# ehsankharazmi/hp-VPINNs

Hardware: AMD Instinct MI355X
Metric: variational-loss iterations/sec (higher is better)
Workload: dtype f64; 1 GPU; Poisson-2D hp-VPINN, 16x16 elements, 20x20 GLL quad/elem, 10x10 test fcns/elem, MLP [2,20,20,20,1] tanh, var_form 1, 320 boundary pts, TF1 Adam (BASELINE config 4); points=102400, residuals=25600, params=921, backend=mfma, parallelism=element-sharded dp1, exchange=none, pass_structure=whole-iteration, kernel_variant=k_iter_fused<L=3,SPLIT=false,QT=true>

## Files before the change

### hp_vpinns_amd/csrc/kernels_fused.hip

```cpp
#include <cstdio>
#include <cstdlib>
#include <cstring>
#include <type_traits>

#include "hpv_mfma_dev.h"
#include "hpv_fused_dev.h"

#define FZ_WAVES 4
#define FZ_BLOCK (FZ_WAVES * 64)
#define FZ_PRE_PER_THREAD 4
#define FZ_C 3
#define FZ_SHAPE_CONSTS                                                                                              \
    static constexpr int FZ_QX = QX_, FZ_QY = QY_, FZ_NTX = NTX_, FZ_NTY = NTY_, FZ_NQ = QX_ * QY_, FZ_NR = NTX_ * NTY_; \
    static constexpr int FZ_TPE = FZ_NQ / 16;                                                                        \
    static constexpr int FZ_MAXT = FZ_TPE / 4 + 1;       \
    static_assert(FZ_NQ % 16 == 0 && FZ_TPE % 4 <= 1, "element shape not covered by the whole-iteration kernel");
#define FZ_SHAPES(X) X(20, 20, 10, 10) X(16, 16, 8, 8) X(12, 12, 6, 6)

#ifdef HPV_FZ_TIMING
#define FZ_STAMP(I) fz_t[I] = clock64()
#define FZ_SEG(I) do { const long long t_ = clock64(); fz_seg[I] += t_ - fz_last; fz_last = t_; } while (0)
#else
#define FZ_STAMP(I)
#define FZ_SEG(I)
// ... 517 lines not shown
        fwd_trip(k0, std::integral_constant<int, 2>{}, std::true_type{});
    } else {
#pragma unroll 1
        for (; k0 + 1 < n_own; k0 += 2) fwd_trip(k0, std::integral_constant<int, 2>{}, std::false_type{});
        if (k0 < n_own) fwd_trip(k0, std::integral_constant<int, 1>{}, std::false_type{});
    }
    FZ_STAMP(2);
    if constexpr (SPLIT) {
        constexpr int NITG = (2 * FZ_NQ * 2 + FZ_BLOCK - 1) / FZ_BLOCK;
        bool ok = true;
        if (!xstay) ok = xg_gather<NITG, FZ_BLOCK>(g.xg + el * (2 * FZ_NQ) * 2, 2 * FZ_NQ * 2, xtag, (unsigned*)(lds + M::CH), tid);
        const int timed_out = __syncthreads_or(ok ? 0 : 1);
        if (timed_out || xstay) {
            if (timed_out && tid == 0) __hip_atomic_store(g.xerr, 1, __ATOMIC_RELAXED, __HIP_MEMORY_SCOPE_AGENT);
            return;
        }
    }
    __syncthreads();
    FZ_STAMP(3);
    if constexpr (QT) {
        if (tid == 0 && dtile < g.ntiles)
            g.data_part[dtile - g.data_off / 16] = (lds[M::RED + 8] + lds[M::RED + 9]) + (lds[M::RED + 10] + lds[M::RED + 11]);
    }

    {
        int nax_e = FZ_NTX, nay_e = FZ_NTY;
        double nr_e = (double)rnr;
        if (pa.pd.nact) {
            nax_e = __builtin_amdgcn_readfirstlane(pa.pd.nact[e]);
            nay_e = __builtin_amdgcn_readfirstlane(pa.pd.nacty[e]);
            nr_e = (double)(nax_e * nay_e);
        }
        constexpr bool PJ_SCALAR = NT2 > 0 && FZ_NQ == 256;
        if constexpr (PJ_SCALAR) {
            static_assert(!GEN || (M::AX == M::TR && 4 <= M::TR_WAVE), "the d-epsilon partials live in wave 0's part of the transpose region (it reads them back itself)");
            for (int o = tid; o < 2 * FZ_QY * FZ_NTX; o += FZ_BLOCK) {
                const int t = o / (FZ_QY * FZ_NTX), j = (o / FZ_NTX) % FZ_QY, r = o % FZ_NTX;
                const double* ax = lds + M::AX + (t * FZ_NTX + r) * FZ_QX;
                const double* gr = lds + M::CH + t * FZ_NQ + j * FZ_QX;
                double acc = 0.0;
#pragma unroll
                for (int i = 0; i < FZ_QX; ++i) acc = fma(ax[i], gr[i], acc);
                lds[M::T + o] = acc;
            }
            __syncthreads();
            if (tid < 2 * FZ_NR) {
                const int t = tid / FZ_NR, o = tid % FZ_NR, kk = o / FZ_NTX, r = o % FZ_NTX;
                const double* by = lds + M::BY + (t * FZ_NTY + kk) * FZ_QY;
                const double* tt = lds + M::T + t * FZ_QY * FZ_NTX + r;
                double acc = 0.0;
#pragma unroll
                for (int j = 0; j < FZ_QY; ++j) acc = fma(by[j], tt[j * FZ_NTX], acc);
                lds[M::UP + tid] = (t == 0 ? pc0 : pc1) * acc;
            }
            __syncthreads();
            double sq = 0.0;
            const double sc = 2.0 / nr_e;
            [[maybe_unused]] double deps = 0.0;
            if (tid < FZ_NR) {
                const bool act = ro_r < nax_e && ro_k < nay_e;
                double u;
                if constexpr (GEN) {
                    const double u0 = lds[M::UP + tid], u1 = lds[M::UP + FZ_NR + tid];
                    u = fma(gm0, u0, gm1 * u1) - pF;
                    if (!act) u = 0.0;
                    deps = sc * u * fma(ge0, u0, ge1 * u1);
                } else {
                    u = (lds[M::UP + tid] + lds[M::UP + FZ_NR + tid]) - pF;
                    if (!act) u = 0.0;
                }
                lds[M::U + tid] = u;
                if (ro_on) pa.R[ro_idx] = u;
                sq = u * u;
            }
            if (wv < 2) {
                sq = group_sum<64>(sq);
                if (lane == 0) lds[M::RED + wv] = sq;
            }
            __syncthreads();
            if (tid == 0) pa.loss_e[e] = (lds[M::RED] + lds[M::RED + 1]) / nr_e;
            for (int o = tid; o < 2 * FZ_NTY * FZ_QX; o += FZ_BLOCK) {
                const int t = o / (FZ_NTY * FZ_QX), kk = (o / FZ_QX) % FZ_NTY, i = o % FZ_QX;
                const double* ax = lds + M::AX + t * FZ_NTX * FZ_QX + i;
                const double* ur = lds + M::U + kk * FZ_NTX;
                double acc = 0.0;
#pragma unroll
                for (int r = 0; r < FZ_NTX; ++r) acc = fma(ax[r * FZ_QX], ur[r], acc);
                if constexpr (GEN) lds[M::S + o] = acc * sc * (t == 0 ? pc0 * gm0 : pc1 * gm1);
                else lds[M::S + o] = acc * sc * (t == 0 ? pc0 : pc1);
            }
            __syncthreads();
            const int n_adj = (GEN && !gtwo) ? FZ_NQ : 2 * FZ_NQ;
            for (int o = tid; o < n_adj; o += FZ_BLOCK) {
                const int t = o / FZ_NQ, j = (o / FZ_QX) % FZ_QY, i = o % FZ_QX;
                const double* by = lds + M::BY + t * FZ_NTY * FZ_QY + j;
                const double* sr = lds + M::S + t * FZ_NTY * FZ_QX + i;
                double acc = 0.0;
#pragma unroll
                for (int kk = 0; kk < FZ_NTY; ++kk) acc = fma(by[kk * FZ_QY], sr[kk * FZ_QX], acc);
                if constexpr (GEN) { if (!gtwo) deps = fma(acc, lds[M::CH + FZ_NQ + o], deps); }
                lds[M::CH + o] = acc;
            }
            if constexpr (GEN) {
                if (pa.pd.has_eps) {
                    deps = group_sum<64>(deps);
                    if (lane == 0) lds[M::AX + wv] = deps;
                }
            }
            __syncthreads();
            if constexpr (GEN) {
                if (pa.pd.has_eps && tid == 0) pa.deps_e[e] = (lds[M::AX] + lds[M::AX + 1]) + (lds[M::AX + 2] + lds[M::AX + 3]);
            }
        } else {
            constexpr int PJ_NJT = (FZ_QY + 15) / 16, PJ_NIT = (FZ_QX + 15) / 16;
            constexpr int PJ_KX = FZ_QX / 4, PJ_KR = (FZ_NTX + 3) / 4, PJ_KK = (FZ_NTY + 3) / 4;
            static_assert(FZ_QX % 4 == 0 && FZ_QY % 4 == 0 && FZ_NTX <= 16 && FZ_NTY <= 16, "projection tiles: whole k-steps over the points, one tile of test functions");
            static_assert(2 * PJ_NJT * FZ_NR <= 2 * FZ_QY * FZ_NTX, "the partial sums of U fit the T array (T itself stays in registers)");
            for (int u = wv; u < 2 * PJ_NJT; u += FZ_WAVES) {
                const int t = u / PJ_NJT, jt = u % PJ_NJT;
                const bool jon = jt * 16 + pt < FZ_QY, ron = pt < FZ_NTX, kon = pt < FZ_NTY;
                const double* gr = lds + M::CH + t * FZ_NQ + (jon ? jt * 16 + pt : 0) * FZ_QX + q;
                const double* ax = lds + M::AX + (t * FZ_NTX + (ron ? pt : 0)) * FZ_QX + q;
                const double* by = lds + M::BY + (t * FZ_NTY + (kon ? pt : 0)) * FZ_QY + jt * 16 + q;
                double ga[PJ_KX], xa[PJ_KX], ya[4];
#pragma unroll
                for (int s = 0; s < PJ_KX; ++s) { ga[s] = gr[4 * s]; xa[s] = ax[4 * s]; }
#pragma unroll
                for (int v = 0; v < 4; ++v) ya[v] = by[jt * 16 + 4 * v < FZ_QY ? 4 * v : 0];
                v4d tt = v4d{0.0, 0.0, 0.0, 0.0};
#pragma unroll
                for (int s = 0; s < PJ_KX; ++s)
                    tt = __builtin_amdgcn_mfma_f64_16x16x4f64(jon ? ga[s] : 0.0, ron ? xa[s] : 0.0, tt, 0, 0, 0);
                v4d up = v4d{0.0, 0.0, 0.0, 0.0};
#pragma unroll
                for (int v = 0; v < 4; ++v)
                    if (jt * 16 + 4 * v < FZ_QY)
                        up = __builtin_amdgcn_mfma_f64_16x16x4f64(kon ? ya[v] : 0.0, tt[v], up, 0, 0, 0);
#pragma unroll
                for (int v = 0; v < 4; ++v)
                    if (q + 4 * v < FZ_NTY && ron) lds[M::T + u * FZ_NR + (q + 4 * v) * FZ_NTX + pt] = up[v];
            }
            pj_lds_barrier();
            double sq = 0.0;
            const double sc = 2.0 / nr_e;
            [[maybe_unused]] double deps = 0.0;
            auto up_t = [&](int t) -> double {
                double a = lds[M::T + t * PJ_NJT * FZ_NR + tid];
#pragma unroll
                for (int jt = 1; jt < PJ_NJT; ++jt) a += lds[M::T + (t * PJ_NJT + jt) * FZ_NR + tid];
                return a;
            };
            if (tid < FZ_NR) {
                const bool act = ro_r < nax_e && ro_k < nay_e;
                double u;
                if constexpr (GEN) {
                    const double u0 = pc0 * up_t(0), u1 = pc1 * up_t(1);
                    u = fma(gm0, u0, gm1 * u1) - pF;
                    if (!act) u = 0.0;
                    deps = sc * u * fma(ge0, u0, ge1 * u1);
                } else {
                    u = (pc0 * up_t(0) + pc1 * up_t(1)) - pF;
                    if (!act) u = 0.0;
                }
                lds[M::U + tid] = u;
                if (ro_on) pa.R[ro_idx] = u;
                sq = u * u;
            }
            if (wv < 2) {
                sq = group_sum<64>(sq);
                if (lane == 0) lds[M::RED + wv] = sq;
            }
            pj_lds_barrier();
            if (tid == 0) pa.loss_e[e] = (lds[M::RED] + lds[M::RED + 1]) / nr_e;
            const int n_adj = (GEN && !gtwo) ? PJ_NIT : 2 * PJ_NIT;
            for (int u = wv; u < n_adj; u += FZ_WAVES) {
                const int t = u / PJ_NIT, it = u % PJ_NIT;
                const int i = it * 16 + pt;
                const bool ion = i < FZ_QX, kon = pt < FZ_NTY;
                const double* ur = lds + M::U + (kon ? pt : 0) * FZ_NTX;
                const double* ax = lds + M::AX + t * FZ_NTX * FZ_QX + (ion ? i : 0);
                double ua[PJ_KR], xa[PJ_KR];
#pragma unroll
                for (int s = 0; s < PJ_KR; ++s) {
                    const int rc = 4 * s + q < FZ_NTX ? 4 * s + q : 0;
                    ua[s] = ur[rc]; xa[s] = ax[rc * FZ_QX];
                }
                v4d ss = v4d{0.0, 0.0, 0.0, 0.0};
#pragma unroll
                for (int s = 0; s < PJ_KR; ++s) {
                    const bool ron = 4 * s + q < FZ_NTX;
                    ss = __builtin_amdgcn_mfma_f64_16x16x4f64((kon && ron) ? ua[s] : 0.0, (ron && ion) ? xa[s] : 0.0, ss, 0, 0, 0);
                }
#pragma unroll
                for (int v = 0; v < 4; ++v) {
                    if constexpr (GEN) ss[v] = ss[v] * sc * (t == 0 ? pc0 * gm0 : pc1 * gm1);
                    else ss[v] = ss[v] * sc * (t == 0 ? pc0 : pc1);
                }
#pragma unroll
                for (int jt = 0; jt < PJ_NJT; ++jt) {
                    const int j = jt * 16 + pt;
                    const bool jon = j < FZ_QY;
                    const double* by = lds + M::BY + t * FZ_NTY * FZ_QY + (jon ? j : 0);
                    v4d gg = v4d{0.0, 0.0, 0.0, 0.0};
#pragma unroll
                    for (int v = 0; v < PJ_KK; ++v) {
                        const bool k4 = 4 * v + q < FZ_NTY;
                        const double b = by[(k4 ? 4 * v + q : 0) * FZ_QY];
                        gg = __builtin_amdgcn_mfma_f64_16x16x4f64((k4 && jon) ? b : 0.0, ss[v], gg, 0, 0, 0);
                    }
#pragma unroll
                    for (int v = 0; v < 4; ++v) {
                        const int jo = jt * 16 + q + 4 * v;
                        if (jo < FZ_QY && ion) {
                            const int o = jo * FZ_QX + i;
                            if constexpr (GEN) { if (!gtwo) deps = fma(gg[v], lds[M::CH + FZ_NQ + o], deps); }
                            lds[M::CH + t * FZ_NQ + o] = gg[v];
                        }
                    }
                }
            }
            if constexpr (GEN) {
                if (pa.pd.has_eps) {
                    deps = group_sum<64>(deps);
                    if (lane == 0) lds[M::UP + wv] = deps;
                }
            }
            __syncthreads();
            if constexpr (GEN) {
                constexpr int PJ_DW = (M::UP - M::TR) / M::TR_WAVE;
                static_assert(PJ_DW < FZ_WAVES && M::UP + FZ_WAVES - M::TR <= (PJ_DW + 1) * M::TR_WAVE, "the d-epsilon partials live in one wave's part of the transpose region");
                if (pa.pd.has_eps && tid == PJ_DW * 64) pa.deps_e[e] = (lds[M::UP] + lds[M::UP + 1]) + (lds[M::UP + 2] + lds[M::UP + 3]);
            }
        }
    }

    FZ_STAMP(4);
    double* TAB = lds + M::TR + wv * M::TR_WAVE;
#pragma unroll
    for (int i = 0; i < LH; ++i) { dWacc[i] = v4d{0.0, 0.0, 0.0, 0.0}; dS10[i] = 0.0; dS01[i] = 0.0; accC[i] = 0.0; }
    dbo = 0.0;
#pragma unroll
    for (int s = 0; s < MF_KS; ++s) {
        dWo[s] = 0.0; dW1[0][s] = 0.0; dW1[1][s] = 0.0;
#pragma unroll
        for (int i = 0; i < L; ++i) db[i][s] = 0.0;
    }

#ifdef HPV_FZ_TIMING
    fz_last = clock64();
    fz_n_own = n_own;
    for (int i = 0; i < 2 + 2 * L; ++i) fz_seg[i] = 0;
#endif
    auto rev_tile = [&](int k) {
#ifdef HPV_FZ_TIMING
        fz_last = clock64();
#endif
        const long tile = tile_of(k);
        const long p = tile * 16 + pt;
        const bool valid = p < g.N;
        const double x0 = valid ? g.X[p] : 0.0, x1 = valid ? g.X[g.N + p] : 0.0;
        int lofs = lane;
        asm volatile("" : "+v"(lofs));
        double sv[NSV];
        if (k < n_lds) {
            const double* pk = k == 0 ? PKw : PKw2;
            if constexpr (NT2 > 0) pk = lds + M::PK + (k == 0 ? wv : (k == 1 ? 4 + wv : 8 + (wv & 1))) * (NSV * 64) + lane;
#pragma unroll
            for (int j = 0; j < NSV; ++j) sv[j] = pk[j * 64];
        } else {
            switch (k - n_lds) {
#define FZ_FETCH(K) case K: if constexpr (K < NREG) acc_get_all<AFULL + K * 2 * NSV, NSV>(sv); break;
                case 0:
                    if constexpr (NREG < 1) {
                    } else if constexpr (NPART > 0) {
                        const double* pp = lds + M::PP + wv * (NPART * 64) + lane;
#pragma unroll
                        for (int j = 0; j < NPART; ++j) sv[j] = pp[j * 64];
                        acc_get_from<ABASE, NSV, NPART>(sv);
                    } else {
                        acc_get_all<ABASE, NSV>(sv);
                    }
                    break;
                FZ_FETCH(1) FZ_FETCH(2) FZ_FETCH(3) FZ_FETCH(4)
#undef FZ_FETCH
                default:
#pragma unroll
                    for (int j = 0; j < NSV; ++j) sv[j] = 0.0;
            }
        }
        double gb[C];
        if (k < n_el) {
            const int lp = (tbase + wv + k * FZ_WAVES) * 16 + pt;
            gb[0] = 0.0; gb[1] = lds[M::CH + lp]; gb[2] = lds[M::CH + FZ_NQ + lp];
            if constexpr (GEN) {
                const double g0 = gb[1], g1 = gb[2];
#pragma unroll
                for (int c = 1; c < C; ++c) gb[c] = fma(wa0(c), g0, wb1(c) * g1);
            }
        } else {
            gb[0] = gdat; gb[1] = 0.0; gb[2] = 0.0;
            if constexpr (NT2 > 0) gb[3] = 0.0;
        }
        if constexpr (NT2 == 0) {
        double zd[L][MF_KS];
#pragma unroll
        for (int s = 0; s < MF_KS; ++s)
            zd[0][s] = fma(gb[1], lds[M::W1O + (0 * MF_KS + s) * 64 + lofs], gb[2] * lds[M::W1O + (1 * MF_KS + s) * 64 + lofs]);
#pragma unroll
        for (int i = 1; i < L; ++i) {
            double hd[MF_KS];
#pragma unroll
            for (int s = 0; s < MF_KS; ++s) {
                const double a = sv[(i - 1) * MF_KS + s];
                hd[s] = (1.0 - a * a) * zd[i - 1][s];
            }
            fz_layer<false>(lds + M::WT + (i - 1) * MF_KS * 64, lds + M::WR + (i - 1) * MF_KS * 16, nullptr, lofs, hd, zd[i]);
        }

        FZ_SEG(0);
        double hbar[2][MF_KS], zbar[2][MF_KS];
#pragma unroll
        for (int s = 0; s < MF_KS; ++s) {
            const double a = sv[(L - 1) * MF_KS + s], a1 = 1.0 - a * a;
            const double wo = lds[M::W1O + (2 * MF_KS + s) * 64 + lofs];
            if (k >= n_el) dWo[s] = fma(a, gb[0], dWo[s]);
            dWo[s] = fma(a1, zd[L - 1][s], dWo[s]);
            hbar[0][s] = gb[0] * wo; hbar[1][s] = wo;
        }
        if (q == 0) dbo += gb[0];
        FZ_SEG(1);

#pragma unroll
        for (int i = L - 1; i >= 0; --i) {
#pragma unroll
            for (int s = 0; s < MF_KS; ++s) {
                const double a = sv[i * MF_KS + s];
                const double a1 = 1.0 - a * a, a2 = -2.0 * a * a1;
                zbar[1][s] = hbar[1][s] * a1;
                const double zb = hbar[0][s] * a1 + a2 * (hbar[1][s] * zd[i][s]);
                zbar[0][s] = zb;
                db[i][s] += zb;
            }
            if (i == 0) {
#pragma unroll
                for (int s = 0; s < MF_KS; ++s) {
                    dW1[0][s] += x0 * zbar[0][s] + gb[1] * zbar[1][s];
                    dW1[1][s] += x1 * zbar[0][s] + gb[2] * zbar[1][s];
                }
            } else {
                pj_wave_sync();
#pragma unroll
                for (int ch = 0; ch < 2; ++ch) {
                    double* TA = TAB + (2 * ch) * (MF_TRB * MF_LD);
                    double* TB = TA + MF_TRB * MF_LD;
#pragma unroll
                    for (int s = 0; s < MF_KS; ++s) {
                        const double a = sv[(i - 1) * MF_KS + s], a1 = 1.0 - a * a;
                        const double hv = ch == 0 ? a : a1 * zd[i - 1][s];
                        TA[(4 * s + q) * MF_LD + pt] = hv;
                        TB[(4 * s + q) * MF_LD + pt] = zbar[ch][s];
                    }
                }
#pragma unroll
                for (int ch = 0; ch < 2; ++ch) {
                    v4d acc = v4d{0.0, 0.0, 0.0, 0.0};
                    double h4 = 0.0;
                    const double* wrl = lds + M::WRB + (i - 1) * MF_KS * 16 + q * 4 + (lane & 3);
#pragma unroll
                    for (int s = 0; s < MF_KS; ++s) {
                        acc = __builtin_amdgcn_mfma_f64_16x16x4f64(lds[M::WN + ((i - 1) * MF_KS + s) * 64 + lofs], zbar[ch][s], acc, 0, 0, 0);
                        h4 = __builtin_amdgcn_mfma_f64_4x4x4f64(wrl[s * 16], zbar[ch][s], h4, 0, 0, 0);
                    }
#pragma unroll
                    for (int s = 0; s < 4; ++s) hbar[ch][s] = acc[s];
                    hbar[ch][4] = h4;
                }
                FZ_SEG(2 + 2 * (L - 1 - i));
                pj_wave_sync();
#pragma unroll
                for (int ch = 0; ch < 2; ++ch) {
                    const double* TA = TAB + (2 * ch) * (MF_TRB * MF_LD);
                    const double* TB = TA + MF_TRB * MF_LD;
                    double aF[4], bF[4], aS[4], bS[4];
#pragma unroll
                    for (int kk = 0; kk < 4; ++kk) {
                        aF[kk] = TA[pt * MF_LD + 4 * kk + q];
                        bF[kk] = TB[pt * MF_LD + 4 * kk + q];
                        aS[kk] = TA[(16 + (lane & 3)) * MF_LD + 4 * kk + q];
                        bS[kk] = TB[(16 + (lane & 3)) * MF_LD + 4 * kk + q];
                    }
#pragma unroll
                    for (int kk = 0; kk < 4; ++kk) {
                        dWacc[i - 1] = __builtin_amdgcn_mfma_f64_16x16x4f64(aF[kk], bF[kk], dWacc[i - 1], 0, 0, 0);
                        dS10[i - 1] = __builtin_amdgcn_mfma_f64_4x4x4f64(aS[kk], bF[kk], dS10[i - 1], 0, 0, 0);
                        dS01[i - 1] = __builtin_amdgcn_mfma_f64_4x4x4f64(bS[kk], aF[kk], dS01[i - 1], 0, 0, 0);
                    }
                    accC[i - 1] = __builtin_amdgcn_mfma_f64_4x4x4f64(TA[(16 + (lane & 3)) * MF_LD + (pt & 12) + q],
                                                                   TB[(16 + (lane & 3)) * MF_LD + (pt & 12) + q], accC[i - 1], 0, 0, 0);
                }
                FZ_SEG(3 + 2 * (L - 1 - i));
            }
        }
        } else {
        double zc[L][2][MF_KS];
        [[maybe_unused]] double zq[L][MF_KS];
        [[maybe_unused]] auto sq2 = [&](int i, int s) -> double { return fma(g.t2w[0], zc[i][0][s] * zc[i][0][s], g.t2w[1] * (zc[i][1][s] * zc[i][1][s])); };
#define ZC(I, CC, SS) zc[(I)][(CC)][(SS)]
#pragma unroll
        for (int s = 0; s < MF_KS; ++s) {
            zc[0][0][s] = lds[M::W1O + (0 * MF_KS + s) * 64 + lofs];
            zc[0][1][s] = lds[M::W1O + (1 * MF_KS + s) * 64 + lofs];
        }
#pragma unroll
        for (int i = 1; i < L; ++i) {
            double hx[MF_KS], hy[MF_KS];
            [[maybe_unused]] double hq[MF_KS];
#pragma unroll
            for (int s = 0; s < MF_KS; ++s) {
                const double a = sv[(i - 1) * MF_KS + s], a1 = 1.0 - a * a;
                hx[s] = a1 * ZC(i - 1, 0, s); hy[s] = a1 * ZC(i - 1, 1, s);
                if constexpr (NT2 > 0) hq[s] = (-2.0 * a * a1) * sq2(i - 1, s) + (i > 1 ? a1 * zq[i > 1 ? i - 1 : 0][s] : 0.0);
            }
            fz_layer<false>(lds + M::WT + (i - 1) * MF_KS * 64, lds + M::WR + (i - 1) * MF_KS * 16, nullptr, lofs, hx, zc[i][0]);
            fz_layer<false>(lds + M::WT + (i - 1) * MF_KS * 64, lds + M::WR + (i - 1) * MF_KS * 16, nullptr, lofs, hy, zc[i][1]);
            if constexpr (NT2 > 0) fz_layer<false>(lds + M::WT + (i - 1) * MF_KS * 64, lds + M::WR + (i - 1) * MF_KS * 16, nullptr, lofs, hq, zq[i]);
        }

        FZ_SEG(0);
        double hbar[C][MF_KS], zbar[C][MF_KS];
        [[maybe_unused]] auto hv3 = [&](int i, int s) -> double {
            const double a = sv[i * MF_KS + s], a1 = 1.0 - a * a;
            return (-2.0 * a * a1) * sq2(i, s) + (i > 0 ? a1 * zq[i][s] : 0.0);
        };
#pragma unroll
        for (int s = 0; s < MF_KS; ++s) {
            const double a = sv[(L - 1) * MF_KS + s], a1 = 1.0 - a * a;
            const double wo = lds[M::W1O + (2 * MF_KS + s) * 64 + lofs];
            if (k >= n_el) dWo[s] = fma(a, gb[0], dWo[s]);
            dWo[s] = fma(a1 * zc[L - 1][0][s], gb[1], dWo[s]);
            dWo[s] = fma(a1 * zc[L - 1][1][s], gb[2], dWo[s]);
            hbar[0][s] = gb[0] * wo; hbar[1][s] = gb[1] * wo; hbar[2][s] = gb[2] * wo;
            if constexpr (NT2 > 0) { dWo[s] = fma(hv3(L - 1, s), gb[3], dWo[s]); hbar[3][s] = gb[3] * wo; }
        }
        if (q == 0) dbo += gb[0];
        FZ_SEG(1);

#pragma unroll
        for (int i = L - 1; i >= 0; --i) {
#pragma unroll
            for (int s = 0; s < MF_KS; ++s) {
                const double a = sv[i * MF_KS + s];
                const double a1 = 1.0 - a * a, a2 = -2.0 * a * a1;
                zbar[1][s] = hbar[1][s] * a1;
                zbar[2][s] = hbar[2][s] * a1;
                double zb = hbar[0][s] * a1 + a2 * (hbar[1][s] * ZC(i, 0, s) + hbar[2][s] * ZC(i, 1, s));
                if constexpr (NT2 > 0) {
                    const double hb = hbar[3][s], a3 = -2.0 * a1 * (1.0 - 3.0 * a * a);
                    zbar[3][s] = hb * a1;
                    zbar[1][s] = fma(2.0 * hb * a2 * g.t2w[0], ZC(i, 0, s), zbar[1][s]);
                    zbar[2][s] = fma(2.0 * hb * a2 * g.t2w[1], ZC(i, 1, s), zbar[2][s]);
                    zb = fma(hb, a3 * sq2(i, s) + (i > 0 ? a2 * zq[i][s] : 0.0), zb);
                }
                zbar[0][s] = zb;
                db[i][s] += zb;
            }
            if (i == 0) {
#pragma unroll
                for (int s = 0; s < MF_KS; ++s) {
                    dW1[0][s] += x0 * zbar[0][s] + zbar[1][s];
                    dW1[1][s] += x1 * zbar[0][s] + zbar[2][s];
                }
            } else {
                pj_wave_sync();
                auto tr_put = [&](int c0) {
#pragma unroll
                    for (int cc = 0; cc < TRG; ++cc) {
                        const int ch = c0 + cc;
                        double* TA = TAB + (2 * cc) * (MF_TRB * MF_LD);
                        double* TB = TA + MF_TRB * MF_LD;
#pragma unroll
                        for (int s = 0; s < MF_KS; ++s) {
                            const double a = sv[(i - 1) * MF_KS + s], a1 = 1.0 - a * a;
                            double hv;
                            if constexpr (NT2 > 0) hv = ch == 0 ? a : (ch == 3 ? hv3(i - 1, s) : a1 * ZC(i - 1, ch == 3 ? 0 : ch - 1, s));
                            else hv = ch == 0 ? a : a1 * ZC(i - 1, ch - 1, s);
                            TA[(4 * s + q) * MF_LD + pt] = hv;
                            TB[(4 * s + q) * MF_LD + pt] = zbar[ch][s];
                        }
                    }
                };
                tr_put(0);
#pragma unroll
                for (int ch = 0; ch < C; ++ch) {
                    v4d acc = v4d{0.0, 0.0, 0.0, 0.0};
                    double h4 = 0.0;
                    const double* wrl = lds + M::WRB + (i - 1) * MF_KS * 16 + q * 4 + (lane & 3);
#pragma unroll
                    for (int s = 0; s < MF_KS; ++s) {
                        acc = __builtin_amdgcn_mfma_f64_16x16x4f64(lds[M::WN + ((i - 1) * MF_KS + s) * 64 + lofs], zbar[ch][s], acc, 0, 0, 0);
                        h4 = __builtin_amdgcn_mfma_f64_4x4x4f64(wrl[s * 16], zbar[ch][s], h4, 0, 0, 0);
                    }
#pragma unroll
                    for (int s = 0; s < 4; ++s) hbar[ch][s] = acc[s];
                    hbar[ch][4] = h4;
                }
                FZ_SEG(2 + 2 * (L - 1 - i));
                pj_wave_sync();
                auto tr_mul = [&]() {
#pragma unroll
                    for (int ch = 0; ch < TRG; ++ch) {
                        const double* TA = TAB + (2 * ch) * (MF_TRB * MF_LD);
                        const double* TB = TA + MF_TRB * MF_LD;
                        double aF[4], bF[4], aS[4], bS[4];
#pragma unroll
                        for (int kk = 0; kk < 4; ++kk) {
                            aF[kk] = TA[pt * MF_LD + 4 * kk + q];
                            bF[kk] = TB[pt * MF_LD + 4 * kk + q];
                            aS[kk] = TA[(16 + (lane & 3)) * MF_LD + 4 * kk + q];
                            bS[kk] = TB[(16 + (lane & 3)) * MF_LD + 4 * kk + q];
                        }
#pragma unroll
                        for (int kk = 0; kk < 4; ++kk) {
                            dWacc[i - 1] = __builtin_amdgcn_mfma_f64_16x16x4f64(aF[kk], bF[kk], dWacc[i - 1], 0, 0, 0);
                            dS10[i - 1] = __builtin_amdgcn_mfma_f64_4x4x4f64(aS[kk], bF[kk], dS10[i - 1], 0, 0, 0);
                            dS01[i - 1] = __builtin_amdgcn_mfma_f64_4x4x4f64(bS[kk], aF[kk], dS01[i - 1], 0, 0, 0);
                        }
                        accC[i - 1] = __builtin_amdgcn_mfma_f64_4x4x4f64(TA[(16 + (lane & 3)) * MF_LD + (pt & 12) + q],
                                                                       TB[(16 + (lane & 3)) * MF_LD + (pt & 12) + q], accC[i - 1], 0, 0, 0);
                    }
                };
                tr_mul();
#pragma unroll
                for (int c0 = TRG; c0 < C; c0 += TRG) {
                    pj_wave_sync();
                    tr_put(c0);
                    pj_wave_sync();
                    tr_mul();
                }
                FZ_SEG(3 + 2 * (L - 1 - i));
            }
        }
        }
        FZ_SEG(1 + 2 * L);
    };
#undef ZC
#pragma unroll 1
    for (int k = 0; k < n_own; ++k) rev_tile(k);

    if constexpr (QT) {
        int lofs = lane;
        asm volatile("" : "+v"(lofs));
        const double X0 = g.X[q_p], X1 = g.X[g.N + q_p];
        double AAq[NSV];
#pragma unroll
        for (int j = 0; j < NSV; ++j) AAq[j] = PKQ[j * 32 + q_ci];
        const double mval = q_tan ? 0.0 : 1.0;
        double gch = lds[M::CH + (q_tan ? (qcs - 1) * FZ_NQ : 0) + q_lp];
        if constexpr (GEN && !DQ) {
            const double g0 = lds[M::CH + q_lp], g1 = lds[M::CH + FZ_NQ + q_lp];
            gch = qcs == 1 ? fma(wa0(1), g0, wb1(1) * g1) : fma(wa0(2), g0, wb1(2) * g1);
        }
        const double GB = q_tan ? (DQ ? 0.0 : gch) : (qcs == 3 ? gdat_q : 0.0);
        double Hq[L][MF_KS], ZCq[L][MF_KS];
#pragma unroll
        for (int s = 0; s < MF_KS; ++s) {
            const double w0 = lds[M::W1O + (0 * MF_KS + s) * 64 + lofs], w1 = lds[M::W1O + (1 * MF_KS + s) * 64 + lofs];
            const double a = AAq[s];
            ZCq[0][s] = qcs == 1 ? w0 : (qcs == 2 ? w1 : 0.0);
            const double ht = (1.0 - a * a) * ZCq[0][s];
            Hq[0][s] = q_tan ? ht : a;
        }
#pragma unroll
        for (int i = 1; i < L; ++i) {
#pragma unroll
            for (int s = 0; s < MF_KS; ++s) {
                const double a = AAq[i * MF_KS + s];
                const double zr = PKZ[((i - 1) * MF_KS + s) * 32 + q_cz];
                const double zc = q_tan ? zr : 0.0;
                const double ht = (1.0 - a * a) * zc;
                ZCq[i][s] = zc;
                Hq[i][s] = q_tan ? ht : a;
            }
        }
        double HB[MF_KS], ZB[MF_KS];
#pragma unroll
        for (int s = 0; s < MF_KS; ++s) {
            const double wo = lds[M::W1O + (2 * MF_KS + s) * 64 + lofs];
            dWo[s] = fma(Hq[L - 1][s], GB, dWo[s]);
            HB[s] = GB * wo;
        }
        dbo += (q == 0 && qcs == 3) ? GB : 0.0;
#pragma unroll
        for (int i = L - 1; i >= 0; --i) {
#pragma unroll
            for (int s = 0; s < MF_KS; ++s) {
                const double a = AAq[i * MF_KS + s];
                const double a1 = 1.0 - a * a, a2 = -2.0 * a * a1;
                const double t = HB[s] * ZCq[i][s];
                const double t4 = dpp_move<0x104>(t), t8 = dpp_move<0x108>(t);
                const double zb = fma(a2 * mval, t4 + t8, HB[s] * a1);
                ZB[s] = zb;
                db[i][s] = fma(mval, zb, db[i][s]);
            }
            if (i == 0) {
                const double c0 = q_tan ? (qcs == 1 ? 1.0 : 0.0) : X0, c1 = q_tan ? (qcs == 2 ? 1.0 : 0.0) : X1;
#pragma unroll
                for (int s = 0; s < MF_KS; ++s) {
                    dW1[0][s] = fma(c0, ZB[s], dW1[0][s]);
                    dW1[1][s] = fma(c1, ZB[s], dW1[1][s]);
                }
            } else {
                pj_wave_sync();
                double* TA = TAB;
                double* TB = TA + MF_TRB * MF_LD;
#pragma unroll
                for (int s = 0; s < MF_KS; ++s) {
                    TA[(4 * s + q) * MF_LD + pt] = Hq[i - 1][s];
                    TB[(4 * s + q) * MF_LD + pt] = ZB[s];
                }
                {
                    v4d acc = v4d{0.0, 0.0, 0.0, 0.0};
                    double h4 = 0.0;
                    const double* wrl = lds + M::WRB + (i - 1) * MF_KS * 16 + q * 4 + (lane & 3);
#pragma unroll
                    for (int s = 0; s < MF_KS; ++s) {
                        acc = __builtin_amdgcn_mfma_f64_16x16x4f64(lds[M::WN + ((i - 1) * MF_KS + s) * 64 + lofs], ZB[s], acc, 0, 0, 0);
                        h4 = __builtin_amdgcn_mfma_f64_4x4x4f64(wrl[s * 16], ZB[s], h4, 0, 0, 0);
                    }
#pragma unroll
                    for (int s = 0; s < 4; ++s) HB[s] = acc[s];
                    HB[4] = h4;
                }
                pj_wave_sync();
                double aF[4], bF[4], aS[4], bS[4];
#pragma unroll
                for (int kk = 0; kk < 4; ++kk) {
                    aF[kk] = TA[pt * MF_LD + 4 * kk + q];
                    bF[kk] = TB[pt * MF_LD + 4 * kk + q];
                    aS[kk] = TA[(16 + (lane & 3)) * MF_LD + 4 * kk + q];
                    bS[kk] = TB[(16 + (lane & 3)) * MF_LD + 4 * kk + q];
                }
#pragma unroll
                for (int kk = 0; kk < 4; ++kk) {
                    dWacc[i - 1] = __builtin_amdgcn_mfma_f64_16x16x4f64(aF[kk], bF[kk], dWacc[i - 1], 0, 0, 0);
                    dS10[i - 1] = __builtin_amdgcn_mfma_f64_4x4x4f64(aS[kk], bF[kk], dS10[i - 1], 0, 0, 0);
                    dS01[i - 1] = __builtin_amdgcn_mfma_f64_4x4x4f64(bS[kk], aF[kk], dS01[i - 1], 0, 0, 0);
                }
                accC[i - 1] = __builtin_amdgcn_mfma_f64_4x4x4f64(TA[(16 + (lane & 3)) * MF_LD + (pt & 12) + q],
                                                               TB[(16 + (lane & 3)) * MF_LD + (pt & 12) + q], accC[i - 1], 0, 0, 0);
            }
        }
// ... 844 lines not shown
```

Baseline: 20460 it/s.

## Stage forward layer inputs in LDS early to shorten backward dW path

For the L=3 non-split kernel, each hidden layer's activations and tangent inputs are written to the per-wave transpose region during the forward pass. In the backward pass, those operands and the transpose weights are prefetched into registers before the zbar computation. Only zbar then has to be transposed through LDS per layer, and the weight-gradient MFMAs use the prefetched operands. This removes one LDS store/sync phase per backward layer. In exchange it holds more registers live across the backward pass and uses more LDS per wave.

New measurement: 20830 it/s, median of 6. 1.02x the previous value.

```diff
diff --git a/hp_vpinns_amd/csrc/kernels_fused.hip b/hp_vpinns_amd/csrc/kernels_fused.hip
--- a/hp_vpinns_amd/csrc/kernels_fused.hip
+++ b/hp_vpinns_amd/csrc/kernels_fused.hip
@@ -843,6 +843,10 @@
             if constexpr (NT2 > 0) gb[3] = 0.0;
         }
         if constexpr (NT2 == 0) {
+        constexpr bool DWE = L == 3 && !SPLIT;
+        constexpr int TRT = MF_TRB * MF_LD;
+        static_assert(!DWE || (2 + 2 * LH) * TRT <= M::TR_WAVE, "the inputs of every hidden layer and one layer's zbar fit the per-wave transpose region");
+        if constexpr (DWE) pj_wave_sync();
         double zd[L][MF_KS];
 #pragma unroll
         for (int s = 0; s < MF_KS; ++s)
@@ -856,7 +860,16 @@
                 hd[s] = (1.0 - a * a) * zd[i - 1][s];
             }
             fz_layer<false>(lds + M::WT + (i - 1) * MF_KS * 64, lds + M::WR + (i - 1) * MF_KS * 16, nullptr, lofs, hd, zd[i]);
-        }
+            if constexpr (DWE) {
+                double* TA = TAB + (2 + 2 * (i - 1)) * TRT;
+#pragma unroll
+                for (int s = 0; s < MF_KS; ++s) {
+                    TA[(4 * s + q) * MF_LD + pt] = sv[(i - 1) * MF_KS + s];
+                    TA[TRT + (4 * s + q) * MF_LD + pt] = hd[s];
+                }
+            }
+        }
+        if constexpr (DWE) pj_wave_sync();
 
         FZ_SEG(0);
         double hbar[2][MF_KS], zbar[2][MF_KS];
@@ -873,6 +886,22 @@
 
 #pragma unroll
         for (int i = L - 1; i >= 0; --i) {
+            [[maybe_unused]] double wn[MF_KS], wr[MF_KS], aF[2][4], aS[2][4], aC[2];
+            if (DWE && i > 0) {
+                const double* wrl = lds + M::WRB + (i - 1) * MF_KS * 16 + q * 4 + (lane & 3);
+#pragma unroll
+                for (int s = 0; s < MF_KS; ++s) { wn[s] = lds[M::WN + ((i - 1) * MF_KS + s) * 64 + lofs]; wr[s] = wrl[s * 16]; }
+#pragma unroll
+                for (int ch = 0; ch < 2; ++ch) {
+                    const double* TA = TAB + (2 + 2 * (i - 1) + ch) * TRT;
+#pragma unroll
+                    for (int kk = 0; kk < 4; ++kk) {
+                        aF[ch][kk] = TA[pt * MF_LD + 4 * kk + q];
+                        aS[ch][kk] = TA[(16 + (lane & 3)) * MF_LD + 4 * kk + q];
+                    }
+                    aC[ch] = TA[(16 + (lane & 3)) * MF_LD + (pt & 12) + q];
+                }
+            }
 #pragma unroll
             for (int s = 0; s < MF_KS; ++s) {
                 const double a = sv[i * MF_KS + s];
@@ -888,6 +917,51 @@
                     dW1[0][s] += x0 * zbar[0][s] + gb[1] * zbar[1][s];
                     dW1[1][s] += x1 * zbar[0][s] + gb[2] * zbar[1][s];
                 }
+            } else if constexpr (DWE) {
+#pragma unroll
+                for (int ch = 0; ch < 2; ++ch) {
+                    double* TB = TAB + ch * TRT;
+#pragma unroll
+                    for (int s = 0; s < MF_KS; ++s) TB[(4 * s + q) * MF_LD + pt] = zbar[ch][s];
+                }
+                pj_wave_sync();
+                double bF[2][4], bS[2][4], bC[2];
+#pragma unroll
+                for (int ch = 0; ch < 2; ++ch) {
+                    const double* TB = TAB + ch * TRT;
+#pragma unroll
+                    for (int kk = 0; kk < 4; ++kk) {
+                        bF[ch][kk] = TB[pt * MF_LD + 4 * kk + q];
+                        bS[ch][kk] = TB[(16 + (lane & 3)) * MF_LD + 4 * kk + q];
+                    }
+                    bC[ch] = TB[(16 + (lane & 3)) * MF_LD + (pt & 12) + q];
+                }
+                pj_wave_sync();
+#pragma unroll
+                for (int ch = 0; ch < 2; ++ch) {
+                    v4d acc = v4d{0.0, 0.0, 0.0, 0.0};
+                    double h4 = 0.0;
+#pragma unroll
+                    for (int s = 0; s < MF_KS; ++s) {
+                        acc = __builtin_amdgcn_mfma_f64_16x16x4f64(wn[s], zbar[ch][s], acc, 0, 0, 0);
+                        h4 = __builtin_amdgcn_mfma_f64_4x4x4f64(wr[s], zbar[ch][s], h4, 0, 0, 0);
+                    }
+#pragma unroll
+                    for (int s = 0; s < 4; ++s) hbar[ch][s] = acc[s];
+                    hbar[ch][4] = h4;
+                }
+                FZ_SEG(2 + 2 * (L - 1 - i));
+#pragma unroll
+                for (int ch = 0; ch < 2; ++ch) {
+#pragma unroll
+                    for (int kk = 0; kk < 4; ++kk) {
+                        dWacc[i - 1] = __builtin_amdgcn_mfma_f64_16x16x4f64(aF[ch][kk], bF[ch][kk], dWacc[i - 1], 0, 0, 0);
+                        dS10[i - 1] = __builtin_amdgcn_mfma_f64_4x4x4f64(aS[ch][kk], bF[ch][kk], dS10[i - 1], 0, 0, 0);
+                        dS01[i - 1] = __builtin_amdgcn_mfma_f64_4x4x4f64(bS[ch][kk], aF[ch][kk], dS01[i - 1], 0, 0, 0);
+                    }
+                    accC[i - 1] = __builtin_amdgcn_mfma_f64_4x4x4f64(aC[ch], bC[ch], accC[i - 1], 0, 0, 0);
+                }
+                FZ_SEG(3 + 2 * (L - 1 - i));
             } else {
                 pj_wave_sync();
 #pragma unroll
```
